# UBCMOCCA/mocca_envs

Hardware: AMD Instinct MI355X
Metric: env-steps/sec, Walker3DCustomEnv-v0 @ 4096 envs, 1/2/4/8 MI355X (higher is better)
Workload: dtype f32; 1 GPU; Walker3DCustomEnv-v0, 4096 envs/GPU, flat ground, U(-1,1) action tape, auto-reset; max_rows=48, max_contacts=12, envs_per_gpu=4096, parallelism=independent env shards x1, no collective, preroll_steps=5912

## Files before the change

### include/mocca.h

```cpp
#ifndef MOCCA_H
#define MOCCA_H

#include <stddef.h>
#include <stdint.h>

#include "mocca_model.h"

#ifdef __cplusplus
extern "C" {
#endif

#define MOCCA_ABI_VERSION 8

typedef struct mocca_ctx *mocca_handle;

enum {
  MOCCA_OK = 0,
  MOCCA_E_ARG = -1,
  MOCCA_E_HIP = -2,
  MOCCA_E_TOPOLOGY = -3,
  MOCCA_E_NODEVICE = -4,
};

enum {
  MOCCA_PARAM_AUTO_RESET = 0,
  MOCCA_PARAM_EVAL_MODE = 1,
  MOCCA_PARAM_CURRICULUM = 2,
  MOCCA_PARAM_RANDOM_POSE = 3,
  MOCCA_PARAM_HOST_RETARGET = 4,
  MOCCA_PARAM_SEED = 5,
  MOCCA_PARAM_ENV_OFFSET = 6,
  MOCCA_PARAM_RANDOM_REWARD = 8,
  MOCCA_PARAM_APPLIED_GAIN = 7,
  MOCCA_PARAM_ISSUE_PRIORITY = 9,
  MOCCA_PARAM_PERSIST_IMPULSES = 10,
  MOCCA_PARAM_KERNEL_VARIANT = 11,
  MOCCA_PARAM_ORDER_EVERY = 12,
  MOCCA_PARAM_PACE_TICKS = 13,
};

#define MOCCA_DEBUG_WORDS 20
enum {
  MOCCA_DBG_ROWS = 0,
  MOCCA_DBG_LIMIT_ROWS = 1,
  MOCCA_DBG_CONTACTS = 2,
  MOCCA_DBG_SLOTS_LO = 3,
  MOCCA_DBG_SLOTS_HI = 4,
  MOCCA_DBG_LIMITS_LO = 5,
  MOCCA_DBG_LIMITS_HI = 6,
  MOCCA_DBG_SELF = 7,
  MOCCA_DBG_CLAMP_LO = 8,
  MOCCA_DBG_CLAMP_HI = 9,
  MOCCA_DBG_CLAMPSIG_LO = 10,
  MOCCA_DBG_CLAMPSIG_HI = 11,
  MOCCA_DBG_CAP_CONTACTS = 12,
  MOCCA_DBG_CAP_ROWS = 13,
  MOCCA_DBG_SUBSTEPS = 14,
  MOCCA_DBG_ROWS_WANTED = 15,
  MOCCA_DBG_STEPSIG_LO = 16,
  MOCCA_DBG_STEPSIG_HI = 17,
  MOCCA_DBG_STEPSIG_N = 18,
  MOCCA_DBG_RESERVED = 19,
};

int mocca_abi_version(void);
size_t mocca_model_sizeof(void);

int mocca_create(const void *model_blob, size_t nbytes, int task_id, int n_envs, int device, mocca_handle *out);
int mocca_destroy(mocca_handle h);

int mocca_n_envs(mocca_handle h);
int mocca_obs_dim(mocca_handle h);
int mocca_act_dim(mocca_handle h);
int mocca_plan_dim(mocca_handle h);
int mocca_state_dim(mocca_handle h);

int mocca_reset(mocca_handle h, const uint8_t *mask_dev, uint64_t seed, float *obs_dev, void *stream);

int mocca_step(mocca_handle h, const float *act_dev, float *obs_dev, float *rew_dev, uint8_t *done_dev,
               int32_t *info_dev, void *stream);

int mocca_task_step(mocca_handle h, const float *act_dev, const int32_t *touch_dev, const int32_t *target_dev,
                    const int32_t *body_dev, float *obs_dev, float *rew_dev, uint8_t *done_dev, int32_t *info_dev,
                    void *stream);

// ... 64 lines not shown
```

### mocca_envs_amd/csrc/mocca_api.hip

```cpp
#include <hip/hip_runtime.h>

#include <cmath>
#include <cstdio>
#include <cstring>
#include <new>
#include <string>
#include <vector>

#include "mocca.h"
#include "mocca_controller.h"
#include "mocca_kernels.h"
#include "mocca_render.h"

using namespace mocca;

extern "C" size_t mocca_r32_args_sizeof(void);
extern "C" int mocca_r32_max_rows(void);
extern "C" int mocca_r32_max_contacts(void);
extern "C" void mocca_r32_launch_step(int topo, int task_id, int n, hipStream_t s, const void* args);
extern "C" void mocca_r32_kernel_info(int topo, int task_id, hipFuncAttributes* fa, int* nb, hipError_t* e);
extern "C" size_t mocca_r64_args_sizeof(void);
extern "C" int mocca_r64_max_rows(void);
extern "C" int mocca_r64_max_contacts(void);
extern "C" void mocca_r64_launch_step(int topo, int task_id, int n, hipStream_t s, const void* args);
// ... 15 lines not shown
  __syncthreads();
  for (int e = t; e < n; e += 1024) {
    const uint32_t r = task[(size_t)e * MOCCA_TASK_WORDS + MOCCA_TW_LAST_ROWS];
    atomicAdd(&hist[63 - (r > 63u ? 63u : r)], 1);
  }
  __syncthreads();
  if (t == 0) {
    int acc = 0;
    for (int k = 0; k < 64; ++k) { start[k] = acc; acc += hist[k]; }
  }
  __syncthreads();
  for (int e = t; e < n; e += 1024) {
    const uint32_t r = task[(size_t)e * MOCCA_TASK_WORDS + MOCCA_TW_LAST_ROWS];
    order[atomicAdd(&start[63 - (r > 63u ? 63u : r)], 1)] = e;
  }
}

struct mocca_ctx {
  MoccaModel model;
  int task_id = 0, n_envs = 0, device = 0, obs_dim = 0;
  MoccaModel* d_model = nullptr;
  int topo = 0;
  float* d_dyn = nullptr;
  uint32_t* d_task = nullptr;
  float* d_terrain = nullptr;
  int auto_reset = 0, eval_mode = 0, random_pose = 1, curriculum = 0, host_retarget = 0, env_offset = 0, random_reward = 0;
  float gain = 1.0f;
  bool compact = false;
  bool wide = false;
  int force_full = 0;
  int persist_warm = 0;
  int pace = -18;
  unsigned long long* d_pace_acc = nullptr;
  float* d_ep_ret = nullptr;
  float *ep_masks = nullptr, *ep_bad = nullptr, *ep_totals = nullptr;
  char* ep_rec = nullptr;
  int ep_slots = 0;
  size_t ep_stride = 0;
  uint32_t ep_serial = 1;
  int order_every = 0;
  int order_age = 0;
  int32_t* d_order = nullptr;
  bool gain_pending = false;
  float* final_obs = nullptr;
  float* d_pvec[3] = {nullptr, nullptr, nullptr};
  bool pvec_on[3] = {false, false, false};
// ... 176 lines not shown
  }
  if (task_id == MOCCA_TASK_WALKER3D_STEPPER &&
      (h->model.n_planks < 1 || h->model.n_planks > MOCCA_MAX_PLANKS || h->model.lookbehind < 1 || h->model.lookbehind > 2)) {
    g_err = "Stepper blob: n_planks must be 1..4 and lookbehind 1 or 2"; delete h; return MOCCA_E_ARG;
  }
  auto fail = [&](const char* what, hipError_t e) {
    g_err = std::string(what) + ": " + hipGetErrorString(e);
    mocca_destroy(h);
    return MOCCA_E_HIP;
  };
  hipError_t e;
  DeviceGuard guard(device);
  if ((e = guard.err) != hipSuccess) return fail("hipSetDevice", e);
  if ((e = hipMalloc(&h->d_model, sizeof(MoccaModel))) != hipSuccess) return fail("hipMalloc(model)", e);
  if ((e = hipMemcpy(h->d_model, &h->model, sizeof(MoccaModel), hipMemcpyHostToDevice)) != hipSuccess) return fail("hipMemcpy(model)", e);
  const size_t dyn_b = (size_t)n_envs * DYN_STRIDE * sizeof(float), task_b = (size_t)n_envs * MOCCA_TASK_WORDS * 4;
  const size_t ter_b = (size_t)n_envs * TERRAIN_STRIDE * sizeof(float);
  if ((e = hipMalloc(&h->d_dyn, dyn_b)) != hipSuccess) return fail("hipMalloc(state)", e);
  if ((e = hipMalloc(&h->d_task, task_b)) != hipSuccess) return fail("hipMalloc(task)", e);
  if ((e = hipMalloc(&h->d_terrain, ter_b)) != hipSuccess) return fail("hipMalloc(terrain)", e);
  if ((e = hipMalloc(&h->d_pace_acc, sizeof(unsigned long long))) != hipSuccess) return fail("hipMalloc(pace samples)", e);
  if ((e = hipMemset(h->d_pace_acc, 0, sizeof(unsigned long long))) != hipSuccess) return fail("hipMemset", e);
  if ((e = hipMemset(h->d_dyn, 0, dyn_b)) != hipSuccess) return fail("hipMemset", e);
  if ((e = hipMemset(h->d_terrain, 0, ter_b)) != hipSuccess) return fail("hipMemset", e);
  {
    uint32_t* tmp = new uint32_t[(size_t)n_envs * MOCCA_TASK_WORDS]();
    const float one = 1.0f;
    uint32_t one_bits; std::memcpy(&one_bits, &one, 4);
    for (int i = 0; i < n_envs; ++i) {
      tmp[(size_t)i * MOCCA_TASK_WORDS + MOCCA_TW_EPISODE] = (uint32_t)-1;
      tmp[(size_t)i * MOCCA_TASK_WORDS + MOCCA_TW_APPLIED_GAIN] = one_bits;
    }
    e = hipMemcpy(h->d_task, tmp, task_b, hipMemcpyHostToDevice);
    delete[] tmp;
    if (e != hipSuccess) return fail("hipMemcpy(task)", e);
  }
  {
    float* tmp = new float[(size_t)n_envs * DYN_STRIDE]();
    for (int i = 0; i < n_envs; ++i) tmp[(size_t)i * DYN_STRIDE + 6] = 1.0f;
    e = hipMemcpy(h->d_dyn, tmp, dyn_b, hipMemcpyHostToDevice);
    delete[] tmp;
    if (e != hipSuccess) return fail("hipMemcpy(state)", e);
  }
  *out = h;
  return MOCCA_OK;
}

int mocca_destroy(mocca_handle h) {
  if (!h) return MOCCA_OK;
  if (h->d_model) (void)hipFree(h->d_model);
  if (h->d_dyn) (void)hipFree(h->d_dyn);
  if (h->d_task) (void)hipFree(h->d_task);
  if (h->d_terrain) (void)hipFree(h->d_terrain);
  if (h->d_traj) (void)hipFree(h->d_traj);
  if (h->d_hf) (void)hipFree(h->d_hf);
  if (h->d_scenes) (void)hipFree(h->d_scenes);
  if (h->d_order) (void)hipFree(h->d_order);
  if (h->d_pace_acc) (void)hipFree(h->d_pace_acc);
  if (h->d_ep_ret) (void)hipFree(h->d_ep_ret);
  for (float* p : h->d_pvec) if (p) (void)hipFree(p);
  if (h->d_ctrl_params) (void)hipFree(h->d_ctrl_params);
  if (h->d_ctrl_layers) (void)hipFree(h->d_ctrl_layers);
  if (h->d_robot_state) (void)hipFree(h->d_robot_state);
  if (h->d_base_act) (void)hipFree(h->d_base_act);
  if (h->d_base_val) (void)hipFree(h->d_base_val);
  delete h;
  return MOCCA_OK;
}

int mocca_n_envs(mocca_handle h) { return h ? h->n_envs : MOCCA_E_ARG; }
int mocca_obs_dim(mocca_handle h) { return h ? h->obs_dim : MOCCA_E_ARG; }
int mocca_act_dim(mocca_handle h) {
  if (!h) return MOCCA_E_ARG;
  return h->task_id == MOCCA_TASK_CASSIE ? h->model.n_ctrl - 2 : h->model.n_joints;
// ... 6 lines not shown
int mocca_state_dim(mocca_handle h) { return h ? MOCCA_STATE_DIM(h->model.n_joints, h->model.n_slots) : MOCCA_E_ARG; }

static StepArgs make_args(mocca_handle h) {
  StepArgs a{};
  a.model = h->d_model; a.dyn = h->d_dyn; a.task = h->d_task; a.terrain = h->d_terrain;
  a.n_envs = h->n_envs; a.obs_dim = h->obs_dim;
  a.auto_reset = h->auto_reset; a.eval_mode = h->eval_mode; a.random_pose = h->random_pose; a.curriculum = h->curriculum;
  a.host_retarget = h->host_retarget; a.env_offset = h->env_offset; a.random_reward = h->random_reward;
  a.seed_lo = (uint32_t)h->seed; a.seed_hi = (uint32_t)(h->seed >> 32);
  a.curriculum_v = h->pvec_on[0] ? h->d_pvec[0] : nullptr;
  a.eval_mode_v = h->pvec_on[1] ? h->d_pvec[1] : nullptr;
  a.gain_v = h->pvec_on[2] ? h->d_pvec[2] : nullptr;
  a.gain = h->gain;
  a.dbg = h->dbg;
  a.prio = h->prio;
  a.traj = h->d_traj; a.traj_n = h->traj_n; a.traj_tmax = h->traj_tmax; a.traj_cstep = h->traj_cstep;
  a.final_obs = h->final_obs;
  a.persist_warm = h->persist_warm;
  a.pace = h->pace;
  a.pace_acc = h->d_pace_acc;
  a.ep_ret = h->d_ep_ret; a.ep_masks = h->ep_masks; a.ep_bad = h->ep_bad; a.ep_totals = h->ep_totals;
  a.hf = h->d_hf; a.hf_rows = h->hf_rows; a.hf_cols = h->hf_cols; a.hf_scale = h->hf_scale;
  a.robot_state = h->d_ctrl_params ? h->d_robot_state : nullptr;
  return a;
}
static int flush_pending(mocca_handle h, hipStream_t s) {
  if (!h->gain_pending) return MOCCA_OK;
  hipLaunchKernelGGL(set_task_word_kernel, dim3((h->n_envs + 255) / 256), dim3(256), 0, s, h->d_task, (int)MOCCA_TW_APPLIED_GAIN, (const float*)nullptr, h->gain, 1, h->n_envs);
  HIP_TRY(h, hipGetLastError());
  h->gain_pending = false;
  return MOCCA_OK;
}
static int need_trajectory(mocca_handle h) {
  if (h->task_id == MOCCA_TASK_CASSIE && h->model.cassie_mode != MOCCA_CASSIE_PLAIN && !h->d_traj) {
    h->err = "this Cassie blob (cassie_mode != 0) needs mocca_set_trajectory before reset / step / observe";
    return MOCCA_E_ARG;
  }
  if (h->task_id == MOCCA_TASK_WALKER3D_PLANNER && !h->d_hf) {
    h->err = "the planner task needs mocca_set_heightfield before reset / step / observe";
    return MOCCA_E_ARG;
  }
  return MOCCA_OK;
}

int mocca_reset(mocca_handle h, const uint8_t* mask_dev, uint64_t seed, float* obs_dev, void* stream) {
  if (!h || !obs_dev) return MOCCA_E_ARG;
  if (need_trajectory(h) != MOCCA_OK) return MOCCA_E_ARG;
  h->seed = seed;
  DeviceGuard guard(h->device);
// ... 310 lines not shown
  StepArgs a = make_args(h);
  a.obs = obs_dev;
  hipStream_t s = (hipStream_t)stream;
  if (int rc = flush_pending(h, s)) return rc;
  dispatch<LaunchObserve>(h->topo, h->task_id, h->n_envs, s, a);
  HIP_TRY(h, hipGetLastError());
  return MOCCA_OK;
}

int mocca_get_state(mocca_handle h, float* state_dev, void* stream) {
  if (!h || !state_dev) return MOCCA_E_ARG;
  DeviceGuard guard(h->device);
  const size_t w = (size_t)mocca_state_dim(h) * sizeof(float);
  HIP_TRY(h, hipMemcpy2DAsync(state_dev, w, h->d_dyn, DYN_STRIDE * sizeof(float), w, h->n_envs, hipMemcpyDeviceToDevice,
                              (hipStream_t)stream));
  return MOCCA_OK;
}
int mocca_set_state(mocca_handle h, const float* state_dev, void* stream) {
  if (!h || !state_dev) return MOCCA_E_ARG;
  DeviceGuard guard(h->device);
  const size_t w = (size_t)mocca_state_dim(h) * sizeof(float);
  HIP_TRY(h, hipMemcpy2DAsync(h->d_dyn, DYN_STRIDE * sizeof(float), state_dev, w, w, h->n_envs, hipMemcpyDeviceToDevice,
                              (hipStream_t)stream));
  return MOCCA_OK;
}
int mocca_get_task(mocca_handle h, uint32_t* task_dev, void* stream) {
  if (!h || !task_dev) return MOCCA_E_ARG;
  DeviceGuard guard(h->device);
  if (int rc = flush_pending(h, (hipStream_t)stream)) return rc;
  HIP_TRY(h, hipMemcpyAsync(task_dev, h->d_task, (size_t)h->n_envs * MOCCA_TASK_WORDS * 4, hipMemcpyDeviceToDevice, (hipStream_t)stream));
  return MOCCA_OK;
}
int mocca_set_task(mocca_handle h, const uint32_t* task_dev, void* stream) {
  if (!h || !task_dev) return MOCCA_E_ARG;
  DeviceGuard guard(h->device);
  h->gain_pending = false;
  HIP_TRY(h, hipMemcpyAsync(h->d_task, task_dev, (size_t)h->n_envs * MOCCA_TASK_WORDS * 4, hipMemcpyDeviceToDevice, (hipStream_t)stream));
  return MOCCA_OK;
}
int mocca_get_terrain(mocca_handle h, float* terrain_dev, void* stream) {
  if (!h || !terrain_dev) return MOCCA_E_ARG;
  DeviceGuard guard(h->device);
  HIP_TRY(h, hipMemcpyAsync(terrain_dev, h->d_terrain, (size_t)h->n_envs * TERRAIN_STRIDE * 4, hipMemcpyDeviceToDevice, (hipStream_t)stream));
  return MOCCA_OK;
}
int mocca_set_terrain(mocca_handle h, const float* terrain_dev, void* stream) {
// ... 18 lines not shown
    case MOCCA_PARAM_ENV_OFFSET: h->env_offset = (int)value; break;
    case MOCCA_PARAM_ISSUE_PRIORITY:
      if (value < 0 || value >= 262144) { h->err = "MOCCA_PARAM_ISSUE_PRIORITY is t1 + 64 t2 + 4096 t3 with each threshold in 0..63"; return MOCCA_E_ARG; }
      h->prio = (int)value;
      break;
    case MOCCA_PARAM_RANDOM_REWARD:
      if (value != 0 && value != 1 && value != 2) { h->err = "MOCCA_PARAM_RANDOM_REWARD is 0, 1 or 2"; return MOCCA_E_ARG; }
      h->random_reward = (int)value; break;
    case MOCCA_PARAM_PERSIST_IMPULSES: h->persist_warm = value != 0; break;
    case MOCCA_PARAM_PACE_TICKS:
      if (value < -64 || value > 1e9) { h->err = "MOCCA_PARAM_PACE_TICKS is a tick count > 0, 0 (off) or -k (self-calibrating, k / 16 of the mean wave time, k <= 64)"; return MOCCA_E_ARG; }
      h->pace = (int)value; break;
    case MOCCA_PARAM_ORDER_EVERY:
      if (value < 0 || value > 1e6) { h->err = "MOCCA_PARAM_ORDER_EVERY is a step count >= 0"; return MOCCA_E_ARG; }
      h->order_every = (int)value; h->order_age = h->order_every;
      if (h->order_every > 0 && !h->d_order) {
        DeviceGuard guard(h->device);
        HIP_TRY(h, hipMalloc(&h->d_order, (size_t)h->n_envs * sizeof(int32_t)));
      }
      break;
    case MOCCA_PARAM_KERNEL_VARIANT:
      if (value != 0 && value != 1 && value != 2) { h->err = "MOCCA_PARAM_KERNEL_VARIANT is 0 (automatic), 1 (force the 48-row instance) or 2 (force the 64-row instance)"; return MOCCA_E_ARG; }
      if (value == 1 && h->wide) { h->err = "MOCCA_PARAM_KERNEL_VARIANT = 1: this blob needs the 64-row instance (caps beyond 48 rows / 12 contacts, or sweep_alternate)"; return MOCCA_E_ARG; }
      h->force_full = (int)value; break;
    default: h->err = "unknown parameter id"; return MOCCA_E_ARG;
  }
  return MOCCA_OK;
}

int mocca_set_param_v(mocca_handle h, int param_id, const float* values_dev, int broadcast, void* stream) {
  if (!h || !values_dev) return MOCCA_E_ARG;
  const int slot = param_id == MOCCA_PARAM_CURRICULUM ? 0 : param_id == MOCCA_PARAM_EVAL_MODE ? 1 : param_id == MOCCA_PARAM_APPLIED_GAIN ? 2 : -1;
  if (slot < 0) { h->err = "this parameter has no per-env form"; return MOCCA_E_ARG; }
  DeviceGuard guard(h->device);
  if (!h->d_pvec[slot]) HIP_TRY(h, hipMalloc(&h->d_pvec[slot], (size_t)h->n_envs * sizeof(float)));
  hipStream_t s = (hipStream_t)stream;
  hipLaunchKernelGGL(copy_param_kernel, dim3((h->n_envs + 255) / 256), dim3(256), 0, s, h->d_pvec[slot], values_dev, broadcast != 0, h->n_envs);
  HIP_TRY(h, hipGetLastError());
  if (slot == 2) {
    h->gain_pending = false;
    hipLaunchKernelGGL(set_task_word_kernel, dim3((h->n_envs + 255) / 256), dim3(256), 0, s, h->d_task, (int)MOCCA_TW_APPLIED_GAIN, (const float*)h->d_pvec[slot], 0.0f, 0, h->n_envs);
    HIP_TRY(h, hipGetLastError());
  }
  h->pvec_on[slot] = true;
  return MOCCA_OK;
}

// ... 81 lines not shown
```

### mocca_envs_amd/csrc/mocca_device.h

```cpp
#pragma once

#include <hip/hip_runtime.h>
#include <stdint.h>

#include "mocca_model.h"
#include "topo_walker3d.h"
#include "topo_cassie.h"
#include "topo_walker2d.h"
#include "topo_crab2d.h"
#include "topo_laikago.h"

#define DI __device__ __forceinline__

#ifndef MOCCA_NS
#define MOCCA_NS mocca
#endif
#ifndef MOCCA_MAXR
#define MOCCA_MAXR 48
#endif
#ifndef MOCCA_COMPACT
#define MOCCA_COMPACT 0
#endif

namespace MOCCA_NS {
// ... 130 lines not shown
  const float* tape;
  int tape_n;
  int32_t* dbg;
  const float* traj;
  int traj_n;
  double traj_tmax, traj_cstep;
  int prio;
  const float* hf;
  int hf_rows, hf_cols;
  float hf_scale;
  float* final_obs;
  int persist_warm;
  const int32_t* order;
  int pace;
  unsigned long long* pace_acc;
  float* ep_ret;
  float* ep_masks;
  float* ep_bad;
  void* ep_rec;
  float* ep_totals;
  uint32_t ep_serial;
  float* robot_state;
  const float* base_value;
};
constexpr int ROBOT_STATE_STRIDE = 64;

DI void wsync() {
  __builtin_amdgcn_fence(__ATOMIC_RELEASE, "wavefront");
  __builtin_amdgcn_wave_barrier();
  __builtin_amdgcn_fence(__ATOMIC_ACQUIRE, "wavefront");
}
DI float dot3(const float* a, const float* b) { return a[0] * b[0] + a[1] * b[1] + a[2] * b[2]; }
DI void cross3(const float* a, const float* b, float* o) {
  float x = a[1] * b[2] - a[2] * b[1], y = a[2] * b[0] - a[0] * b[2], z = a[0] * b[1] - a[1] * b[0];
  o[0] = x; o[1] = y; o[2] = z;
}
DI float dot6(const float* a, const float* b) {
  return a[0] * b[0] + a[1] * b[1] + a[2] * b[2] + a[3] * b[3] + a[4] * b[4] + a[5] * b[5];
}
DI void matvec3(const float* R, const float* x, float* o) {
  float a = R[0] * x[0] + R[1] * x[1] + R[2] * x[2];
  float b = R[3] * x[0] + R[4] * x[1] + R[5] * x[2];
  float c = R[6] * x[0] + R[7] * x[1] + R[8] * x[2];
  o[0] = a; o[1] = b; o[2] = c;
}
DI void matmul3(const float* A, const float* B, float* C) {
// ... 283 lines not shown
        cross3(om, cw, wxc);
        float vc[3] = {v[3] + wxc[0], v[4] + wxc[1], v[5] + wxc[2]};
        const float kl = unif(M->lin_damp) * ms * (1.0f + __builtin_sqrtf(dot3(vc, vc)));
        const float ka = unif(M->ang_damp) * (1.0f + __builtin_sqrtf(dot3(om, om)));
#pragma unroll
        for (int i = 0; i < 3; ++i) F[i] = kl * vc[i];
        cross3(cw, F, cxF);
#pragma unroll
        for (int i = 0; i < 3; ++i) { p[i] += ka * Iom[i] + cxF[i]; p[3 + i] += F[i]; }
      }
#pragma unroll
      for (int i = 0; i < 6; ++i)
#pragma unroll
        for (int jx = 0; jx < 6; ++jx) L[L_M + 36 * b + 6 * i + jx] = I[sym(i, jx)];
#pragma unroll
      for (int i = 0; i < 6; ++i) L[L_P + 6 * b + i] = p[i];
      L[L_SV + SVS * b + SV_INVD] = jarm;
      L[L_SV + SVS * b + SV_UU] = L[L_TAU + b] - jdamp * L[L_QD + b];
    }
  }
}

template <class T, bool FULL>
DI void walk_kinematics(ModelP M, float* L, int lane, unsigned long long ppk) {
  asm volatile("" : "+v"(lane));
  const int b = lane < T::NB ? lane : 0;
  WalkConsts wk;
  walk_consts<FULL>(M, b, wk);
  walk_phase1<T>(L, lane, ppk);
  wsync();
  walk_phase2<T, FULL>(M, L, lane, b, ppk, wk);
}

DI void chol6_factor(const float* A, float* F) {
  float Lm[6][6];
#pragma unroll
  for (int j = 0; j < 6; ++j) {
    float s = A[sym(j, j)];
#pragma unroll
    for (int k = 0; k < j; ++k) s -= Lm[j][k] * Lm[j][k];
    const float id = rsq(s);
    F[sym(j, j)] = id;
#pragma unroll
    for (int i = j + 1; i < 6; ++i) {
      float t = A[sym(i, j)];
#pragma unroll
      for (int k = 0; k < j; ++k) t -= Lm[i][k] * Lm[j][k];
      Lm[i][j] = t * id;
      F[sym(i, j)] = Lm[i][j];
    }
  }
}
// ... 1302 lines not shown
  if (lane < T::NB) {
    const int j = lane;
    float s, cq;
    fast_sincos(L[L_Q + j], &s, &cq);
    const float t = 1.0f - cq;
    float ax[3], jr[9], Rq[9], Tl[9];
#pragma unroll
    for (int i = 0; i < 3; ++i) ax[i] = M->jaxis[j][i];
#pragma unroll
    for (int i = 0; i < 9; ++i) jr[i] = M->jrot[j][i];
    Rq[0] = cq + t * ax[0] * ax[0];          Rq[1] = t * ax[0] * ax[1] - s * ax[2];   Rq[2] = t * ax[0] * ax[2] + s * ax[1];
    Rq[3] = t * ax[0] * ax[1] + s * ax[2];   Rq[4] = cq + t * ax[1] * ax[1];          Rq[5] = t * ax[1] * ax[2] - s * ax[0];
    Rq[6] = t * ax[0] * ax[2] - s * ax[1];   Rq[7] = t * ax[1] * ax[2] + s * ax[0];   Rq[8] = cq + t * ax[2] * ax[2];
    matmul3(jr, Rq, Tl);
    float4* rec = reinterpret_cast<float4*>(L + L_SV + SVS * j);
    rec[0] = make_float4(Tl[0], Tl[1], Tl[2], Tl[3]);
    rec[1] = make_float4(Tl[4], Tl[5], Tl[6], Tl[7]);
    rec[2] = make_float4(Tl[8], M->jpos[j][0], M->jpos[j][1], M->jpos[j][2]);
    rec[3] = make_float4(ax[0], ax[1], ax[2], L[L_QD + j]);
  }
  wsync();
}

template <class T, int TASK>
DI ContactFlags substep(ModelP M, float* L, int lane, const float* ter, int next_step_index,
                        unsigned long long ppk, int32_t* dbg, int prio, int& rows_out,
                        const HeightFieldArgs hfa = HeightFieldArgs{nullptr, 0, 0, 0.0f}, int sidx = 0, int nsub = 1, int* cover_out = nullptr) {
  const int per0 = 64 + MOCCA_PACE_ROWUNIT * rows_out, done0 = sidx * per0, total = nsub * per0;
  STAMP(30);
  stage_joints<T>(M, L, lane);
  STAMP(29);
  int nc = 0, nc_wanted = 0;
  float Afac[21] = {0, 0, 0, 0, 0, 0, 0, 0, 0, 0, 0, 0, 0, 0, 0, 0, 0, 0, 0, 0, 0};
  ContactFlags fl = {0, 0, 0, 0, 0, 0, 0, 0, 0};
  if constexpr (COMPACT) {
    static_assert(!COMPACT || T::NCLOS == 0, "closure rows read the body frames after the ABA: not in the compact layout");
    int wl = lane;
    asm volatile("" : "+v"(wl));
    walk_phase1<T>(L, wl, ppk);
    wsync();
    STAMP(0);
    geom_points<T>(M, L, lane);
    wsync();
    STAMP(15);
#ifndef MOCCA_SKIP_COLLIDE
    fl = collide<T, TASK>(M, L, lane, ter, next_step_index, &nc, dbg, &nc_wanted, hfa, cover_out);
#endif
    wsync();
    const int wb = wl < T::NB ? wl : 0;
    WalkConsts wk;
    walk_consts<true>(M, wb, wk);
    walk_phase2<T, true>(M, L, wl, wb, ppk, wk);
    wsync();
  } else {
    walk_kinematics<T, true>(M, L, lane, ppk);
    wsync();
    STAMP(0);
    geom_points<T>(M, L, lane);
    wsync();
    STAMP(15);
#ifndef MOCCA_SKIP_COLLIDE
    fl = collide<T, TASK>(M, L, lane, ter, next_step_index, &nc, dbg, &nc_wanted, hfa, cover_out);
#endif
  }
  STAMP(1);
  pace_checkpoint(L, done0 + 20, total);
#ifndef MOCCA_SKIP_ABA
  aba_passes<T>(M, L, lane, ppk, Afac);
#endif
  STAMP(2);
  pace_checkpoint(L, done0 + 36, total);
#ifndef MOCCA_SKIP_SOLVE
  solve_constraints<T>(M, L, lane, nc, nc_wanted, ppk, dbg, Afac, prio, rows_out);
#endif
  if (dbg) { __builtin_amdgcn_s_waitcnt(0); dbg_fold_step(dbg, lane); }
  STAMP(3);
#ifdef MOCCA_DUMMY_VALU
  {
// ... 275 lines not shown
        const int mr = M->mirror_right[k], ml = M->mirror_left[k];
        if (k < nms) {
          if (mr == j) src = ml + 1;
          if (ml == j) src = mr + 1;
        }
      }
#pragma unroll
      for (int k = 0; k < 2; ++k) if (k < nmn && M->mirror_neg[k] == j) sgn = -1.0f;
    }
    const float base = sgn * M->init_q[src];
    float qn = base;
    if (a.random_pose) {
      const float ds = -0.1f + 0.2f * draw_u<INJECT>(a, env, t.episode, t.draw + (b - 1));
      const float wt = M->jhi[b] - M->jlo[b], bs = M->jlo[b];
      float ps = 2 * (base + ds - bs) / wt - 1;
      ps = ps < -0.95f ? -0.95f : (ps > 0.95f ? 0.95f : ps);
      qn = wt * (ps + 1) / 2 + bs;
    }
    L[L_Q + b] = qn;
    L[L_QD + b] = 0.0f;
  }
  if (a.random_pose) t.draw += T::NJ;
  reset_base_pose<T>(M, L, lane);
  RobotObs ro = robot_obs<T>(M, L, lane, 0.0f, 0.0f, obs);
  float dist, cd, sd;
  if (TASK == MOCCA_TASK_WALKER3D_PLANNER) {
    const float R = M->target_range;
    const float ux = draw_u<INJECT>(a, env, t.episode, t.draw), uy = draw_u<INJECT>(a, env, t.episode, t.draw + 1);
    t.draw += 2;
    t.wt[0] = -R + 2.0f * R * ux;
    t.wt[1] = -R + 2.0f * R * uy;
    t.wt[2] = hf_height_at(a.hf, a.hf_rows, a.hf_cols, a.hf_scale, t.wt[0], t.wt[1]);
    calc_potential(M, L, t, ro, &dist, &cd, &sd);
    if (lane == 0) softsign_tail(sd, cd, obs + ROBOT_OBS<T>);
  } else if (TASK == MOCCA_TASK_WALKER3D_CUSTOM) {
    calc_potential(M, L, t, ro, &dist, &cd, &sd);
    if (lane == 0) {
      softsign_tail(sd, cd, obs + ROBOT_OBS<T>);
      if (M->task_flags & MOCCA_TASKF_RESET_TAIL_ZERO) { obs[ROBOT_OBS<T>] = 0.0f; obs[ROBOT_OBS<T> + 1] = 0.0f; }
    }
  } else {
    generate_terrain<INJECT>(a, M, env, t, L, ter, lane);
    t.nsi = M->lookbehind;
    delta_to_k_targets(M, L, ter, t, ro, lane, obs + ROBOT_OBS<T>);
    calc_potential(M, L, t, ro, &dist, &cd, &sd);
  }
// ... 172 lines not shown
```

### mocca_envs_amd/csrc/mocca_kernels.h

```cpp
#pragma once
#include <hip/hip_runtime.h>

#include "mocca.h"
#include "mocca_device.h"

namespace MOCCA_NS {

#ifndef MOCCA_WAVES_PER_EU
#define MOCCA_WAVES_PER_EU 4
#endif

DI void flush_obs(const float* L, float* dst, int lane, int obs_dim) {
#pragma unroll 1
  for (int k = lane; k < obs_dim; k += 64) dst[k] = L[L_OBS + k];
}
DI void keep_terminal_obs(const StepArgs& a, const float* L, int env, int lane) {
  wsync();
  if (a.final_obs) flush_obs(L, a.final_obs + (size_t)env * a.obs_dim, lane, a.obs_dim);
  wsync();
}

template <class T>
DI void keep_robot_state(const StepArgs& a, const float* L, int env, int lane) {
  static_assert(ROBOT_OBS<T> <= 64 && ROBOT_OBS<T> <= ROBOT_STATE_STRIDE, "one store per lane");
// ... 201 lines not shown
    rew = cassie_mocap_reward(a, M, L, lane, cs, jv, f1);
  }
  cassie_observe(M, L, lane, cs, t.initz, jv, phase, obs);
  return {rew, 0};
}

template <class T, int TASK, bool INJECT = false>
__global__ __launch_bounds__(64, MOCCA_WAVES_PER_EU) void mocca_step_kernel(StepArgs a) {
  __shared__ float L[L_TOTAL];
  const int lane = threadIdx.x;
  if ((int)blockIdx.x >= a.n_envs) return;
  const int env = a.order ? uni(a.order[blockIdx.x]) : (int)blockIdx.x;
  ModelP M = (ModelP)a.model;
  float* st = a.dyn + (size_t)env * DYN_STRIDE;
  uint32_t* tk = a.task + (size_t)env * MOCCA_TASK_WORDS;
  float* ter = TASK == MOCCA_TASK_WALKER3D_STEPPER ? a.terrain + (size_t)env * TERRAIN_STRIDE : nullptr;
  float* obs_out = a.obs + (size_t)env * a.obs_dim;
  float* obs = L + L_OBS;
  int32_t* dbg = a.dbg ? a.dbg + (size_t)env * MOCCA_DEBUG_WORDS : nullptr;

  const bool warm_ld = INJECT || uni(__float_as_int(M->warmstart)) != 0, warm_st = warm_ld || a.persist_warm != 0;
  if (dbg && lane == 0) { dbg[16] = 0; dbg[17] = 0; dbg[18] = 0; }
  load_dyn(st, L, lane, T::NJ, T::NSLOT, warm_ld);
  pace_start(a, L, lane, INJECT ? 0 : a.pace);
  if (lane == 0) L[L_KEEPWARM] = __int_as_float(warm_st ? 1 : 0);
  const unsigned long long ppk = T::path_packed(lane < T::NB ? lane : 0);
  ContactFlags fl = {0, 0, 0, 0, 0, 0, 0, 0, 0};
  int cover = 0;
  if constexpr (TASK == MOCCA_TASK_CASSIE) {
    const int no = M->n_ordered, nctl = M->n_ctrl, mode = M->cassie_mode;
    float target = 0.0f;
    if (lane < nctl) {
      float base = M->ctrl_base[lane];
      if (mode != MOCCA_CASSIE_PLAIN) {
        const int f0 = traj_frame(a, M, (int)tk[MOCCA_TW_ISTEP]);
        base = (lane < nctl - 2 && M->residual_control) ? a.traj[(size_t)f0 * MOCCA_TRAJ_STRIDE + M->ctrl_oidx[lane]] : 0.0f;
      }
      target = base + (lane < nctl - 2 ? a.act[(size_t)env * (nctl - 2) + lane] : 0.0f);
    }
    if (lane < no) {
      L[L_JVEL + lane] = __uint_as_float(tk[MOCCA_TW_JVEL + lane]);
      L[L_Q0 + lane] = L[L_Q + M->ordered_body[lane]];
    }
    if (lane < MOCCA_MAX_BODIES) L[L_TAU + lane] = 0.0f;
    if (lane == 0) { L[L_Q] = 0.0f; L[L_QD] = 0.0f; }
    wsync();
// ... 27 lines not shown
    {
      const float applied_gain = __uint_as_float(tk[MOCCA_TW_APPLIED_GAIN]);
      if (lane < T::NJ) {
        const float act_raw = a.act[(size_t)env * T::NJ + lane];
        const float c = act_raw < -1.0f ? -1.0f : (act_raw > 1.0f ? 1.0f : act_raw);
        L[L_TAU + 1 + lane] = M->gain[lane + 1] * applied_gain * c;
      }
    }
    if (lane == 0) { L[L_TAU] = 0.0f; L[L_Q] = 0.0f; L[L_QD] = 0.0f; }
    wsync();

    STAMP(28);
    if constexpr (TASK == MOCCA_TASK_WALKER3D_STEPPER) stage_planks(M, L, lane, ter);
    const int nsub = INJECT ? 0 : M->n_substeps;
    const int nsi0 = TASK == MOCCA_TASK_WALKER3D_STEPPER ? (int)tk[MOCCA_TW_NEXT_STEP_INDEX] : 0;
    int last_rows = uni((int)tk[MOCCA_TW_LAST_ROWS]);
    if (!INJECT && a.pace == 0) set_issue_priority(last_rows, a.prio);
#pragma unroll 1
    for (int s = 0; s < nsub; ++s) {
      ModelP Ms = M;
      int ln = lane;
      unsigned long long pk = ppk;
      asm volatile("" : "+s"(Ms), "+v"(ln), "+v"(pk));
      fl = substep<T, TASK>(Ms, L, ln, ter, nsi0, pk, dbg, a.prio, last_rows, HeightFieldArgs{a.hf, a.hf_rows, a.hf_cols, a.hf_scale}, s, nsub, &cover);
    }
    if constexpr (INJECT) {
      const int32_t* tc = a.inj_touch + (size_t)env * T::NFEET;
      fl.touch0 = tc[0] != 0; fl.touch1 = tc[1] != 0;
      if constexpr (T::NFEET > 2) { fl.touch2 = tc[2] != 0; fl.touch3 = tc[3] != 0; }
      if (a.inj_target) {
        const int32_t* tg = a.inj_target + (size_t)env * T::NFEET;
        const int npl = TASK == MOCCA_TASK_WALKER3D_STEPPER ? M->n_planks : 1;
#pragma unroll
        for (int f = 0; f < T::NFEET; ++f)
          if (tg[f] == 1 || tg[f] == 2) cover |= 1 << (4 * f + (nsi0 + tg[f] - 1) % npl);
        fl.target0 = tg[0] == 1; fl.target1 = tg[1] == 1;
        if constexpr (T::NFEET > 2) { fl.target2 = tg[2] == 1; fl.target3 = tg[3] == 1; }
      }
      if (a.inj_body) fl.body_touch = a.inj_body[env] != 0;
    }
    if (!INJECT && lane == 0) tk[MOCCA_TW_LAST_ROWS] = (uint32_t)last_rows;
    STAMP(27);
  }
  TaskRegs t = load_task<T, TASK>(tk);
  const float ep_ret0 = a.ep_ret ? a.ep_ret[env] : 0.0f;
  StepResult r;
  if constexpr (TASK == MOCCA_TASK_CASSIE) r = cassie_step<T>(a, M, L, tk, lane, ppk, t, obs);
// ... 9 lines not shown
    t.t += 1;
    if constexpr (TASK == MOCCA_TASK_WALKER3D_PLANNER) r = planner_step<T>(M, L, lane, t, fl, obs, a.base_value ? a.base_value + env : nullptr);
    else if constexpr (TASK == MOCCA_TASK_WALKER3D_CUSTOM) r = custom_step<T, INJECT>(a, M, L, env, lane, t, fl, act_raw, obs);
    else r = stepper_step<T, INJECT>(a, M, L, ter, tk, env, lane, t, fl, cover, act_raw, obs);
    t.prevx = L[L_BASE];
  }
  const int timeout = t.t >= M->max_episode_steps;
  const int dflag = (t.done ? 1 : 0) | (timeout ? 2 : 0);
  if (lane == 0) {
    a.rew[env] = r.rew;
    a.done[env] = (uint8_t)dflag;
    if (a.info) a.info[env] = r.info;
    if (a.ep_ret) monitor_emit(a, env, ep_ret0, r.rew, dflag, t.t, r.info);
  }
  STAMP(26);
  if (a.auto_reset && dflag) {
    keep_terminal_obs(a, L, env, lane);
    reset_task<T, TASK, INJECT>(a, M, L, ter, tk, env + a.env_offset, lane, t, obs);
  }
  wsync();
  flush_obs(L, obs_out, lane, a.obs_dim);
  if constexpr (TASK == MOCCA_TASK_WALKER3D_PLANNER) keep_robot_state<T>(a, L, env, lane);
  store_dyn(st, L, lane, T::NJ, T::NSLOT, uni(__float_as_int(L[L_KEEPWARM])) != 0);
  if (lane == 0) store_task<T, TASK, true>(tk, t);
  if (!INJECT) pace_finish(a, L, lane, a.pace);
  STAMP(25);
#ifdef MOCCA_STAMPS
  if (lane == 0 && blockIdx.x < STAMP_WAVES) g_stamps[blockIdx.x * STAMP_SLOTS + 24] = (unsigned long long)(a.auto_reset && dflag);
#endif
}

template <class T, int TASK, bool INJECT = false>
__global__ __launch_bounds__(64) void mocca_reset_kernel(StepArgs a) {
  __shared__ float L[L_TOTAL];
  const int env = blockIdx.x, lane = threadIdx.x;
  if (env >= a.n_envs) return;
  if (a.mask && !a.mask[env]) return;
  ModelP M = (ModelP)a.model;
  float* st = a.dyn + (size_t)env * DYN_STRIDE;
  uint32_t* tk = a.task + (size_t)env * MOCCA_TASK_WORDS;
  float* ter = TASK == MOCCA_TASK_WALKER3D_STEPPER ? a.terrain + (size_t)env * TERRAIN_STRIDE : nullptr;
  TaskRegs t = load_task<T, TASK, true>(tk);
  if (lane == 0) { L[L_Q] = 0.0f; L[L_QD] = 0.0f; if (a.ep_ret) a.ep_ret[env] = 0.0f; }
  reset_task<T, TASK, INJECT>(a, M, L, ter, tk, env + a.env_offset, lane, t, L + L_OBS);
  wsync();
  flush_obs(L, a.obs + (size_t)env * a.obs_dim, lane, a.obs_dim);
  if constexpr (TASK == MOCCA_TASK_WALKER3D_PLANNER) keep_robot_state<T>(a, L, env, lane);
  store_dyn(st, L, lane, T::NJ, T::NSLOT);
  if (lane == 0) store_task<T, TASK, true>(tk, t);
}

template <class T, int TASK>
__global__ __launch_bounds__(64) void mocca_observe_kernel(StepArgs a) {
  __shared__ float L[L_TOTAL];
  const int env = blockIdx.x, lane = threadIdx.x;
  if (env >= a.n_envs) return;
  ModelP M = (ModelP)a.model;
  const float* st = a.dyn + (size_t)env * DYN_STRIDE;
  uint32_t* tk = a.task + (size_t)env * MOCCA_TASK_WORDS;
  const float* ter = TASK == MOCCA_TASK_WALKER3D_STEPPER ? a.terrain + (size_t)env * TERRAIN_STRIDE : nullptr;
  float* obs = L + L_OBS;
  load_dyn(st, L, lane, T::NJ, T::NSLOT);
  TaskRegs t = load_task<T, TASK>(tk);
  if (lane == 0) { L[L_Q] = 0.0f; L[L_QD] = 0.0f; }
  wsync();
  stage_joints<T>(M, L, lane);
  walk_kinematics<T, false>(M, L, lane, T::path_packed(lane < T::NB ? lane : 0));
  wsync();
  if constexpr (TASK == MOCCA_TASK_CASSIE) {
    const CassieState cs = cassie_state(M, L, lane, t.initz);
    float phase = 0.0f;
    if (M->cassie_mode != MOCCA_CASSIE_PLAIN) traj_frame(a, M, t.istep, &phase);
    cassie_observe(M, L, lane, cs, t.initz, lane < MOCCA_MAX_CTRL ? __uint_as_float(tk[MOCCA_TW_JVEL + lane]) : 0.0f, phase, obs);
    t.linpot = cassie_potential(M, L);
  } else {
    RobotObs ro = robot_obs<T>(M, L, lane, t.fc0, t.fc1, obs, t.fc2, t.fc3);
    float dist, cd, sd;
    if (TASK == MOCCA_TASK_WALKER3D_CUSTOM || TASK == MOCCA_TASK_WALKER3D_PLANNER) {
      calc_potential(M, L, t, ro, &dist, &cd, &sd);
      if (lane == 0) softsign_tail(sd, cd, obs + ROBOT_OBS<T>);
    } else {
      delta_to_k_targets(M, L, ter, t, ro, lane, obs + ROBOT_OBS<T>);
      calc_potential(M, L, t, ro, &dist, &cd, &sd);
    }
    t.prevx = L[L_BASE];
  }
  wsync();
  flush_obs(L, a.obs + (size_t)env * a.obs_dim, lane, a.obs_dim);
  if constexpr (TASK == MOCCA_TASK_WALKER3D_PLANNER) keep_robot_state<T>(a, L, env, lane);
  if (lane == 0) store_task<T, TASK>(tk, t);
}
// ... 31 lines not shown
```

### mocca_envs_amd/lib.py

```python
from __future__ import annotations

import ctypes as C
import os

HERE = os.path.dirname(os.path.abspath(__file__))
LIB_PATH = os.environ.get("MOCCA_LIB_PATH") or os.path.join(HERE, "libmocca_hip.so")

ABI_VERSION = 8
PARAM_AUTO_RESET, PARAM_EVAL_MODE, PARAM_CURRICULUM, PARAM_RANDOM_POSE, PARAM_HOST_RETARGET, PARAM_SEED, PARAM_ENV_OFFSET, PARAM_APPLIED_GAIN, PARAM_RANDOM_REWARD = 0, 1, 2, 3, 4, 5, 6, 7, 8
PARAM_ISSUE_PRIORITY = 9
PARAM_PERSIST_IMPULSES = 10
PARAM_KERNEL_VARIANT = 11
PARAM_ORDER_EVERY = 12
PARAM_PACE_TICKS = 13
DEBUG_WORDS = 20
CAMERA_FLOATS = 16
RENDER_MAX_SIZE = 4096
RENDER_ID_NONE, RENDER_ID_GROUND, RENDER_ID_PLANK0, RENDER_ID_HEIGHTFIELD, RENDER_ID_TARGET, RENDER_ID_LINK0 = -1, 32, 33, 37, 38, 64

_vp, _i, _u64, _sz, _d = C.c_void_p, C.c_int, C.c_uint64, C.c_size_t, C.c_double
SYMBOLS = {
    "mocca_abi_version": (_i, []),
    "mocca_model_sizeof": (_sz, []),
    "mocca_create": (_i, [_vp, _sz, _i, _i, _i, C.POINTER(_vp)]),
    "mocca_destroy": (_i, [_vp]),
    "mocca_n_envs": (_i, [_vp]),
    "mocca_obs_dim": (_i, [_vp]),
    "mocca_act_dim": (_i, [_vp]),
    "mocca_plan_dim": (_i, [_vp]),
    "mocca_state_dim": (_i, [_vp]),
    "mocca_reset": (_i, [_vp, _vp, _u64, _vp, _vp]),
    "mocca_step": (_i, [_vp, _vp, _vp, _vp, _vp, _vp, _vp]),
    "mocca_task_step": (_i, [_vp] * 10),
    "mocca_set_base_controller": (_i, [_vp, _vp, _sz, _vp, _i, _d]),
    "mocca_plan_step": (_i, [_vp, _vp, _vp, _vp, _vp, _vp, _vp]),
    "mocca_get_base_outputs": (_i, [_vp, _vp, _vp, _vp]),
    "mocca_set_draw_tape": (_i, [_vp, _vp, _i]),
# ... 60 lines not shown
```

Baseline: 41.13 million env-steps/s.

## Carry forward-kinematics frames across steps to skip first-substep recomputation

Adds a per-env global kinematics record (body rotations/translations and joint axes) written at the end of each step, on reset and on observe. The next step reloads it and, for the first substep, skips stage_joints and walk_phase1. The record is invalidated when set_state is called or the kernel variant changes. This removes redundant kinematics work at the start of each step in exchange for extra global memory traffic (about 336 floats per env per step, read and written) and a risk of stale frames if some state path is not invalidated.

```diff
diff --git a/include/mocca.h b/include/mocca.h
--- a/include/mocca.h
+++ b/include/mocca.h
@@ -37,6 +37,7 @@
   MOCCA_PARAM_KERNEL_VARIANT = 11,
   MOCCA_PARAM_ORDER_EVERY = 12,
   MOCCA_PARAM_PACE_TICKS = 13,
+  MOCCA_PARAM_KIN_CARRY = 14,
 };
 
 #define MOCCA_DEBUG_WORDS 20
@@ -60,7 +61,7 @@
   MOCCA_DBG_STEPSIG_LO = 16,
   MOCCA_DBG_STEPSIG_HI = 17,
   MOCCA_DBG_STEPSIG_N = 18,
-  MOCCA_DBG_RESERVED = 19,
+  MOCCA_DBG_KIN_CARRIED = 19,
 };
 
 int mocca_abi_version(void);
diff --git a/mocca_envs_amd/csrc/mocca_api.hip b/mocca_envs_amd/csrc/mocca_api.hip
--- a/mocca_envs_amd/csrc/mocca_api.hip
+++ b/mocca_envs_amd/csrc/mocca_api.hip
@@ -61,6 +61,9 @@
   MoccaModel* d_model = nullptr;
   int topo = 0;
   float* d_dyn = nullptr;
+  float* d_kin = nullptr;
+  int kin_carry = 1;
+  bool kin_stale = false;
   uint32_t* d_task = nullptr;
   float* d_terrain = nullptr;
   int auto_reset = 0, eval_mode = 0, random_pose = 1, curriculum = 0, host_retarget = 0, env_offset = 0, random_reward = 0;
@@ -283,6 +286,9 @@
   if ((e = hipMalloc(&h->d_pace_acc, sizeof(unsigned long long))) != hipSuccess) return fail("hipMalloc(pace samples)", e);
   if ((e = hipMemset(h->d_pace_acc, 0, sizeof(unsigned long long))) != hipSuccess) return fail("hipMemset", e);
   if ((e = hipMemset(h->d_dyn, 0, dyn_b)) != hipSuccess) return fail("hipMemset", e);
+  const size_t kin_b = (size_t)n_envs * KIN_STRIDE * sizeof(float);
+  if ((e = hipMalloc(&h->d_kin, kin_b)) != hipSuccess) return fail("hipMalloc(kinematics)", e);
+  if ((e = hipMemset(h->d_kin, 0, kin_b)) != hipSuccess) return fail("hipMemset", e);
   if ((e = hipMemset(h->d_terrain, 0, ter_b)) != hipSuccess) return fail("hipMemset", e);
   {
     uint32_t* tmp = new uint32_t[(size_t)n_envs * MOCCA_TASK_WORDS]();
@@ -311,6 +317,7 @@
   if (!h) return MOCCA_OK;
   if (h->d_model) (void)hipFree(h->d_model);
   if (h->d_dyn) (void)hipFree(h->d_dyn);
+  if (h->d_kin) (void)hipFree(h->d_kin);
   if (h->d_task) (void)hipFree(h->d_task);
   if (h->d_terrain) (void)hipFree(h->d_terrain);
   if (h->d_traj) (void)hipFree(h->d_traj);
@@ -363,9 +370,17 @@
   a.ep_ret = h->d_ep_ret; a.ep_masks = h->ep_masks; a.ep_bad = h->ep_bad; a.ep_totals = h->ep_totals;
   a.hf = h->d_hf; a.hf_rows = h->hf_rows; a.hf_cols = h->hf_cols; a.hf_scale = h->hf_scale;
   a.robot_state = h->d_ctrl_params ? h->d_robot_state : nullptr;
+  a.kin = h->d_kin; a.kin_carry = h->kin_carry;
   return a;
 }
+static hipError_t invalidate_kin(mocca_handle h, hipStream_t s) {
+  return hipMemset2DAsync(h->d_kin + KIN_VALID, KIN_STRIDE * sizeof(float), 0, sizeof(float), h->n_envs, s);
+}
 static int flush_pending(mocca_handle h, hipStream_t s) {
+  if (h->kin_stale) {
+    HIP_TRY(h, invalidate_kin(h, s));
+    h->kin_stale = false;
+  }
   if (!h->gain_pending) return MOCCA_OK;
   hipLaunchKernelGGL(set_task_word_kernel, dim3((h->n_envs + 255) / 256), dim3(256), 0, s, h->d_task, (int)MOCCA_TW_APPLIED_GAIN, (const float*)nullptr, h->gain, 1, h->n_envs);
   HIP_TRY(h, hipGetLastError());
@@ -722,6 +737,7 @@
   const size_t w = (size_t)mocca_state_dim(h) * sizeof(float);
   HIP_TRY(h, hipMemcpy2DAsync(h->d_dyn, DYN_STRIDE * sizeof(float), state_dev, w, w, h->n_envs, hipMemcpyDeviceToDevice,
                               (hipStream_t)stream));
+  HIP_TRY(h, invalidate_kin(h, (hipStream_t)stream));
   return MOCCA_OK;
 }
 int mocca_get_task(mocca_handle h, uint32_t* task_dev, void* stream) {
@@ -786,7 +802,9 @@
     case MOCCA_PARAM_KERNEL_VARIANT:
       if (value != 0 && value != 1 && value != 2) { h->err = "MOCCA_PARAM_KERNEL_VARIANT is 0 (automatic), 1 (force the 48-row instance) or 2 (force the 64-row instance)"; return MOCCA_E_ARG; }
       if (value == 1 && h->wide) { h->err = "MOCCA_PARAM_KERNEL_VARIANT = 1: this blob needs the 64-row instance (caps beyond 48 rows / 12 contacts, or sweep_alternate)"; return MOCCA_E_ARG; }
+      if (h->force_full != (int)value) h->kin_stale = true;
       h->force_full = (int)value; break;
+    case MOCCA_PARAM_KIN_CARRY: h->kin_carry = value != 0; break;
     default: h->err = "unknown parameter id"; return MOCCA_E_ARG;
   }
   return MOCCA_OK;
diff --git a/mocca_envs_amd/csrc/mocca_device.h b/mocca_envs_amd/csrc/mocca_device.h
--- a/mocca_envs_amd/csrc/mocca_device.h
+++ b/mocca_envs_amd/csrc/mocca_device.h
@@ -176,6 +176,8 @@
   uint32_t ep_serial;
   float* robot_state;
   const float* base_value;
+  float* kin;
+  int kin_carry;
 };
 constexpr int ROBOT_STATE_STRIDE = 64;
 
@@ -505,12 +507,12 @@
 }
 
 template <class T, bool FULL>
-DI void walk_kinematics(ModelP M, float* L, int lane, unsigned long long ppk) {
+DI void walk_kinematics(ModelP M, float* L, int lane, unsigned long long ppk, bool have_frames = false) {
   asm volatile("" : "+v"(lane));
   const int b = lane < T::NB ? lane : 0;
   WalkConsts wk;
   walk_consts<FULL>(M, b, wk);
-  walk_phase1<T>(L, lane, ppk);
+  if (!have_frames) walk_phase1<T>(L, lane, ppk);
   wsync();
   walk_phase2<T, FULL>(M, L, lane, b, ppk, wk);
 }
@@ -1859,13 +1861,39 @@
   wsync();
 }
 
+constexpr int KIN_AXES = 264, KIN_VALID = 328, KIN_STRIDE = 336;
+template <class T>
+DI void store_kin(float* kn, const float* L, int lane) {
+  static_assert(3 * (T::NB - 1) <= 64 && 12 * T::NB <= KIN_AXES && KIN_AXES + 3 * (T::NB - 1) <= KIN_VALID, "kinematics record layout");
+  if (lane < 3 * (T::NB - 1)) {
+    const int g = (lane * 43) >> 7, ri = lane - 3 * g;
+    reinterpret_cast<float4*>(kn)[3 + lane] = *reinterpret_cast<const float4*>(L + L_RT + 12 + 4 * lane);
+    kn[KIN_AXES + lane] = L[L_SV + SVS * (g + 1) + ri];
+  }
+  if (lane < 3) reinterpret_cast<float4*>(kn)[lane] = *reinterpret_cast<const float4*>(L + L_RT + 4 * lane);
+  if (lane == 0) kn[KIN_VALID] = __int_as_float(1);
+}
+template <class T>
+DI void load_kin(const float* kn, float* L, int lane) {
+  if (lane < 3 * (T::NB - 1)) {
+    const int g = (lane * 43) >> 7, ri = lane - 3 * g;
+    *reinterpret_cast<float4*>(L + L_RT + 12 + 4 * lane) = reinterpret_cast<const float4*>(kn)[3 + lane];
+    L[L_SV + SVS * (g + 1) + ri] = kn[KIN_AXES + lane];
+  }
+  if (lane < 3) *reinterpret_cast<float4*>(L + L_RT + 4 * lane) = reinterpret_cast<const float4*>(kn)[lane];
+}
+DI void drop_kin(float* kn, int lane) {
+  if (lane == 0) kn[KIN_VALID] = __int_as_float(0);
+}
+
 template <class T, int TASK>
 DI ContactFlags substep(ModelP M, float* L, int lane, const float* ter, int next_step_index,
                         unsigned long long ppk, int32_t* dbg, int prio, int& rows_out,
-                        const HeightFieldArgs hfa = HeightFieldArgs{nullptr, 0, 0, 0.0f}, int sidx = 0, int nsub = 1, int* cover_out = nullptr) {
+                        const HeightFieldArgs hfa = HeightFieldArgs{nullptr, 0, 0, 0.0f}, int sidx = 0, int nsub = 1, int* cover_out = nullptr,
+                        bool have_frames = false) {
   const int per0 = 64 + MOCCA_PACE_ROWUNIT * rows_out, done0 = sidx * per0, total = nsub * per0;
   STAMP(30);
-  stage_joints<T>(M, L, lane);
+  if (!have_frames) stage_joints<T>(M, L, lane);
   STAMP(29);
   int nc = 0, nc_wanted = 0;
   float Afac[21] = {0, 0, 0, 0, 0, 0, 0, 0, 0, 0, 0, 0, 0, 0, 0, 0, 0, 0, 0, 0, 0};
@@ -1874,7 +1902,7 @@
     static_assert(!COMPACT || T::NCLOS == 0, "closure rows read the body frames after the ABA: not in the compact layout");
     int wl = lane;
     asm volatile("" : "+v"(wl));
-    walk_phase1<T>(L, wl, ppk);
+    if (!have_frames) walk_phase1<T>(L, wl, ppk);
     wsync();
     STAMP(0);
     geom_points<T>(M, L, lane);
@@ -1890,7 +1918,7 @@
     walk_phase2<T, true>(M, L, wl, wb, ppk, wk);
     wsync();
   } else {
-    walk_kinematics<T, true>(M, L, lane, ppk);
+    walk_kinematics<T, true>(M, L, lane, ppk, have_frames);
     wsync();
     STAMP(0);
     geom_points<T>(M, L, lane);
@@ -2212,6 +2240,11 @@
   }
   if (a.random_pose) t.draw += T::NJ;
   reset_base_pose<T>(M, L, lane);
+  {
+    float* kn = a.kin + (size_t)(env - a.env_offset) * KIN_STRIDE;
+    if constexpr (INJECT) drop_kin(kn, lane);
+    else store_kin<T>(kn, L, lane);
+  }
   RobotObs ro = robot_obs<T>(M, L, lane, 0.0f, 0.0f, obs);
   float dist, cd, sd;
   if (TASK == MOCCA_TASK_WALKER3D_PLANNER) {
diff --git a/mocca_envs_amd/csrc/mocca_kernels.h b/mocca_envs_amd/csrc/mocca_kernels.h
--- a/mocca_envs_amd/csrc/mocca_kernels.h
+++ b/mocca_envs_amd/csrc/mocca_kernels.h
@@ -247,6 +247,15 @@
   const bool warm_ld = INJECT || uni(__float_as_int(M->warmstart)) != 0, warm_st = warm_ld || a.persist_warm != 0;
   if (dbg && lane == 0) { dbg[16] = 0; dbg[17] = 0; dbg[18] = 0; }
   load_dyn(st, L, lane, T::NJ, T::NSLOT, warm_ld);
+  bool kin_ok = false;
+  if constexpr (!INJECT && TASK != MOCCA_TASK_CASSIE) {
+    if (a.kin_carry) {
+      const float* kn = a.kin + (size_t)env * KIN_STRIDE;
+      kin_ok = uni(__float_as_int(kn[KIN_VALID])) != 0;
+      load_kin<T>(kn, L, lane);
+    }
+    if (dbg && lane == 0) dbg[MOCCA_DBG_KIN_CARRIED] = kin_ok ? 1 : 0;
+  }
   pace_start(a, L, lane, INJECT ? 0 : a.pace);
   if (lane == 0) L[L_KEEPWARM] = __int_as_float(warm_st ? 1 : 0);
   const unsigned long long ppk = T::path_packed(lane < T::NB ? lane : 0);
@@ -320,7 +329,8 @@
       int ln = lane;
       unsigned long long pk = ppk;
       asm volatile("" : "+s"(Ms), "+v"(ln), "+v"(pk));
-      fl = substep<T, TASK>(Ms, L, ln, ter, nsi0, pk, dbg, a.prio, last_rows, HeightFieldArgs{a.hf, a.hf_rows, a.hf_cols, a.hf_scale}, s, nsub, &cover);
+      fl = substep<T, TASK>(Ms, L, ln, ter, nsi0, pk, dbg, a.prio, last_rows, HeightFieldArgs{a.hf, a.hf_rows, a.hf_cols, a.hf_scale}, s, nsub, &cover,
+                             s == 0 && kin_ok);
     }
     if constexpr (INJECT) {
       const int32_t* tc = a.inj_touch + (size_t)env * T::NFEET;
@@ -376,6 +386,13 @@
   flush_obs(L, obs_out, lane, a.obs_dim);
   if constexpr (TASK == MOCCA_TASK_WALKER3D_PLANNER) keep_robot_state<T>(a, L, env, lane);
   store_dyn(st, L, lane, T::NJ, T::NSLOT, uni(__float_as_int(L[L_KEEPWARM])) != 0);
+  if constexpr (TASK != MOCCA_TASK_CASSIE) {
+    int ek = env;
+    asm volatile("" : "+s"(ek));
+    float* kn = a.kin + (size_t)ek * KIN_STRIDE;
+    if constexpr (INJECT) drop_kin(kn, lane);
+    else if (!(a.auto_reset && dflag)) store_kin<T>(kn, L, lane);
+  }
   if (lane == 0) store_task<T, TASK, true>(tk, t);
   if (!INJECT) pace_finish(a, L, lane, a.pace);
   STAMP(25);
@@ -421,6 +438,7 @@
   stage_joints<T>(M, L, lane);
   walk_kinematics<T, false>(M, L, lane, T::path_packed(lane < T::NB ? lane : 0));
   wsync();
+  if constexpr (TASK != MOCCA_TASK_CASSIE) store_kin<T>(a.kin + (size_t)env * KIN_STRIDE, L, lane);
   if constexpr (TASK == MOCCA_TASK_CASSIE) {
     const CassieState cs = cassie_state(M, L, lane, t.initz);
     float phase = 0.0f;
diff --git a/mocca_envs_amd/lib.py b/mocca_envs_amd/lib.py
--- a/mocca_envs_amd/lib.py
+++ b/mocca_envs_amd/lib.py
@@ -13,6 +13,7 @@
 PARAM_KERNEL_VARIANT = 11
 PARAM_ORDER_EVERY = 12
 PARAM_PACE_TICKS = 13
+PARAM_KIN_CARRY = 14
 DEBUG_WORDS = 20
 CAMERA_FLOATS = 16
 RENDER_MAX_SIZE = 4096
```

Result: no change. 41.37 million env-steps/s, median of 6 (+0.6%).
